# genome/breakdancer

Hardware: AMD Instinct MI355X
Metric: read-pairs/s, records resident in HBM -> scored SV table (SURVEY 8d timing i); end to end from BAM: config.timings.bam_to_table (vs_baseline is taken there) (higher is better)
Workload: dtype int32

## Files before the change

### breakdancer_amd/csrc/k2_compact.hip

```cpp
#include <cstdlib>

#include "bdx_dev.h"
#include "bdx_finalize.h"

namespace bdx {

size_t k2_lds_bytes(int) { return 0; }

constexpr int kSub = kK2TilesPerWave;
constexpr int kPerLane = 4 * kSub;
constexpr int kTile2 = kTile * kSub;
constexpr int kSlice = 256;
constexpr int kOffBits = 10;
static_assert(kPerLane <= 32 && kTile2 <= (1 << kOffBits), "K2 super tile");

__device__ __forceinline__ unsigned class_byte(const uint64_t (&cq)[kSub / 2], int r) {
    uint64_t v = cq[0];
#pragma unroll
    for (int q = 1; q < kSub / 2; ++q) v = (r >> 3) == q ? cq[q] : v;
    return (unsigned)((v >> (8 * (r & 7))) & 255u);
}

__device__ __forceinline__ void key_and_qlen_of(const K2Params& p, uint64_t i, uint64_t& key, int& qlen, uint64_t& check) {
    if (p.nseg == 0) {
// ... 156 lines not shown
                    const uint64_t i = (uint64_t)tile2 * kTile2 + (src & ((1u << kOffBits) - 1u));
                    const uint32_t j = rank0 + win + q;
                    const unsigned sam = p.r.flag[i];
                    p.c.tid[j] = p.r.tid[i];
                    p.c.pos[j] = p.r.pos[i];
                    p.c.isize[j] = abs(p.r.isize[i]);
                    uint64_t key, check = 0;
                    int qlen;
                    key_and_qlen_of(p, i, key, qlen, check);
                    p.c.meta[j] = meta_pack((int)((src >> kOffBits) & 15u), (sam >> 4) & 1u, lib_of(p, i), qlen);
                    p.c.key[j] = key;
                    if (p.c.check) p.c.check[j] = check;
                    p.c.idx[j] = (uint32_t)i;
                    p.c.nn[j] = s_nn[w * kSlice + q];
                }
            }
            __builtin_amdgcn_wave_barrier();
        }
        uint64_t kq[kSub / 2];
#pragma unroll
        for (int q = 0; q < kSub / 2; ++q) kq[q] = 0;
        if (nkeys > 1) {
#pragma unroll
            for (int r = 0; r < kPerLane; ++r)
                if (r < nvalid) kq[r >> 3] |= (uint64_t)(p.libs[lib_of(p, base + r)].key & 255) << (8 * (r & 7));
        }
        for (int k0 = 0; k0 < nkeys; k0 += 2) {
            uint32_t mk0 = 0, mk1 = 0;
            if (nkeys > 1) {
#pragma unroll
                for (int r = 0; r < kPerLane; ++r) {
                    const int key = (int)((kq[r >> 3] >> (8 * (r & 7))) & 255u);
                    if ((m_pk >> r) & 1u) { mk0 |= key == k0 ? 1u << r : 0u; mk1 |= key == k0 + 1 ? 1u << r : 0u; }
                }
            } else {
                mk0 = m_pk;
            }
            const uint32_t v = (uint32_t)__popc(mk0) + ((uint32_t)__popc(mk1) << 16);
            const uint32_t ex = wave_incl_scan(v) - v;
            const uint32_t b0 = k0 == 0 ? pre_k0 : col_prefix<kBases>(p, kColKey0 + k0, tile2, chunk, lane);
            const uint32_t b1 = k0 + 1 < nkeys ? (k0 == 0 ? pre_k1 : col_prefix<kBases>(p, kColKey0 + k0 + 1, tile2, chunk, lane)) : 0u;
            uint32_t j = rank0 + local0;
            for (uint32_t mm = m_anom; mm; mm &= mm - 1, ++j) {
                if (j >= p.c.cap) break;
                const int r = __builtin_ctz(mm);
                const uint32_t upto = (2u << r) - 1u;
                p.c.pk[(size_t)k0 * p.c.cap + j] = b0 + (ex & 0xFFFFu) + (uint32_t)__popc(mk0 & upto);
                if (k0 + 1 < nkeys) p.c.pk[(size_t)(k0 + 1) * p.c.cap + j] = b1 + (ex >> 16) + (uint32_t)__popc(mk1 & upto);
            }
        }
    }
}

__device__ __forceinline__ void k2_fills(const K2Params& p) {
#pragma nounroll
    for (int f = 0; f < 4; ++f)
        for (uint32_t i = blockIdx.x * kBlock + threadIdx.x; i < p.fill_words[f]; i += gridDim.x * kBlock) p.fill_ptr[f][i] = p.fill_value[f];
}

__global__ __launch_bounds__(kBlock) void k2_compact_kernel(const K2Params p) {
    k2_fills(p);
    k2_body<true>(p, gridDim.x);
}

__global__ __launch_bounds__(kBlock) void k2_compact_side_kernel(const K2Params p, const FinalizeParams fp) {
    k2_fills(p);
    if (blockIdx.x == gridDim.x - 1) {
        finalize2_body(fp);
        return;
    }
    k2_body<false>(p, gridDim.x - 1);
}

void launch_k2(const K2Params& p, size_t lds, hipStream_t s, const FinalizeParams* side) {
    const uint32_t ntiles2 = (p.ntiles + kSub - 1) / kSub;
    const uint32_t nblk = (ntiles2 + kWaves - 1) / kWaves;
    const uint32_t cap = 8192u;
    const uint32_t grid = nblk < cap ? nblk : cap;
    if (side) hipLaunchKernelGGL(k2_compact_side_kernel, dim3(grid + 1), dim3(kBlock), lds, s, p, *side);
    else hipLaunchKernelGGL(k2_compact_kernel, dim3(grid), dim3(kBlock), lds, s, p);
}

}

__global__ void k2_noop_kernel() {}
namespace bdx { void warm_k2(hipStream_t s) { hipLaunchKernelGGL(k2_noop_kernel, dim3(1), dim3(64), 0, s); } }
```

### breakdancer_amd/csrc/k4_join.hip

```cpp
#include "bdx_k3.h"
#include "bdx_scan.h"

namespace bdx {

__device__ __forceinline__ uint64_t mix64(uint64_t h) {
    h ^= h >> 33;
    h *= 0xff51afd7ed558ccdull;
    h ^= h >> 33;
    h *= 0xc4ceb9fe1a85ec53ull;
    h ^= h >> 33;
    return h;
}
__device__ __forceinline__ uint32_t bucket_of(uint64_t h, uint32_t log2b) { return log2b ? (uint32_t)(h >> (64 - log2b)) : 0u; }

constexpr int kPartChunk = 512;

__global__ __launch_bounds__(256) void k4_count_kernel(K4Arrays k4, Entries en, const uint32_t* n_ptr) {
    extern __shared__ __attribute__((aligned(16))) unsigned char smem[];
    uint32_t* s_h = (uint32_t*)smem;
    const uint32_t na = *n_ptr;
    const uint32_t base = blockIdx.x * kPartChunk;
    if (base >= na) return;
    for (uint32_t b = threadIdx.x; b < k4.nbuckets; b += 256) s_h[b] = 0;
    __syncthreads();
// ... 66 lines not shown
__device__ __forceinline__ void join_bucket(uint64_t* tkey, int32_t* tidx, uint32_t cap, const K4Arrays& k4, const int32_t* region,
                                            const uint64_t* check, uint32_t off, uint32_t cnt, StageCounts* counts) {
    for (uint32_t s = threadIdx.x; s < cap; s += blockDim.x) tidx[s] = -1;
    __syncthreads();
    for (uint32_t e = threadIdx.x; e < cnt; e += blockDim.x) {
        const uint64_t key = k4.e_key[off + e];
        const int32_t j = (int32_t)k4.e_idx[off + e];
        uint32_t s = (uint32_t)(mix64(key) & 0xffffffffu) % cap;
        uint32_t probes = 0;
        bool placed = true;
        while (atomicCAS(&tidx[s], -1, j) != -1) {
            s = s + 1 == cap ? 0 : s + 1;
            if (++probes > kMaxProbes) { placed = false; break; }
        }
        if (placed) tkey[s] = key;
        else counts->irregular = 1;
    }
    __syncthreads();
    for (uint32_t e = threadIdx.x; e < cnt; e += blockDim.x) {
        const uint64_t key = k4.e_key[off + e];
        const int32_t j = (int32_t)k4.e_idx[off + e];
        uint32_t s = (uint32_t)(mix64(key) & 0xffffffffu) % cap;
        int32_t mate = -1;
        const uint32_t lim = cap < kMaxProbes ? cap : kMaxProbes;
        for (uint32_t probes = 0; probes < lim; ++probes) {
            const int32_t o = tidx[s];
            if (o == -1) break;
            if (o != j && tkey[s] == key && (!check || check[o] == check[j])) {
                if (mate != -1) counts->irregular = 1;
                mate = o;
            }
            s = s + 1 == cap ? 0 : s + 1;
        }
        if (mate >= 0 && (region[j] < 0 || region[mate] < 0)) mate = -2;
        k4.partner[j] = mate;
    }
}

__global__ __launch_bounds__(256) void k4_join_kernel(K4Arrays k4, const int32_t* region, const uint64_t* check, StageCounts* counts) {
    extern __shared__ __attribute__((aligned(16))) unsigned char smem[];
    const uint32_t b = blockIdx.x;
    const uint32_t off = k4.boff[b], cnt = k4.boff[b + 1] - off;
    if (cnt == 0) return;
    if (2 * cnt <= (uint32_t)kJoinLdsSlots) {
        uint64_t* tkey = (uint64_t*)smem;
        int32_t* tidx = (int32_t*)(tkey + kJoinLdsSlots);
        join_bucket<true>(tkey, tidx, 2 * cnt, k4, region, check, off, cnt, counts);
    } else {
        join_bucket<false>(k4.t_key + 2 * (size_t)off, k4.t_idx + 2 * (size_t)off, 2 * cnt, k4, region, check, off, cnt, counts);
    }
}

constexpr uint32_t kJoinForwardBlocks = 32;
__global__ __launch_bounds__(256) void k4_direct_join_kernel(K4Arrays k4, Entries en, const uint32_t* n_ptr, StageCounts* counts) {
    const uint32_t na = *n_ptr;
    const uint32_t fwd = en.r_rec_host ? kJoinForwardBlocks : 0u;
    if (blockIdx.x < fwd) {
        const uint32_t nr = en.counts->n_regions;
        const uint32_t t = blockIdx.x * 256 + threadIdx.x, gsz = fwd * 256;
        constexpr uint32_t kw = sizeof(RegionRec) / 4;
        {
            const uint32_t words = nr * kw, quads = words / 4;
            const uint4* src = (const uint4*)en.r_rec_dev;
            uint4* dst = (uint4*)en.r_rec_host;
            for (uint32_t i = t; i < quads; i += gsz) dst[i] = src[i];
            if (t < words - quads * 4) ((uint32_t*)en.r_rec_host)[quads * 4 + t] = ((const uint32_t*)en.r_rec_dev)[quads * 4 + t];
        }
        {
            const uint32_t words = nr * (uint32_t)en.nkeys2, quads = words / 4;
            const uint4* src = (const uint4*)en.r_pk_dev;
            uint4* dst = (uint4*)en.r_pk_host;
            for (uint32_t i = t; i < quads; i += gsz) dst[i] = src[i];
            if (t < words - quads * 4) en.r_pk_host[quads * 4 + t] = en.r_pk_dev[quads * 4 + t];
        }
    }
    const uint32_t j = blockIdx.x < fwd ? 0xFFFFFFFFu : (blockIdx.x - fwd) * 256 + threadIdx.x;
    const uint32_t kp = (blockIdx.x - fwd) * 4 + (threadIdx.x >> 6);
    (void)kp;
    KPROF(kp, 0);
    KPROF(kp, 1);
    if (j >= na) return;
    const uint32_t nl = en.n_local ? *en.n_local : na;
    const bool jf = j >= nl;
    int rj;
    if (jf) {
        rj = en.fregion[j - nl];
    } else if (en.c_rid) {
        rj = en.c_rid[en.cand[j]];
        en.region_out[j] = rj;
        if (en.k6_scratch) {
            const size_t cap = en.scratch_cap;
            en.k6_scratch[j] = 0; en.k6_scratch[cap + j] = j; en.k6_scratch[2 * cap + j] = 0; en.k6_scratch[3 * cap + j] = 0;
            en.k6_scratch[4 * cap + j] = 0; en.k6_scratch[5 * cap + j] = 0;
        }
    } else {
        rj = en.region[j];
    }
    const uint64_t key = jf ? en.fkey[j - nl] : en.key[j];
    const uint64_t chk = en.check ? (jf ? en.fcheck[j - nl] : en.check[j]) : 0ull;
    const uint64_t h = mix64(key);
    if (key != 0x5555AAAA5555AAAAull) KPROF(kp, 2);
    const uint32_t tag = (uint32_t)(h >> 32);
    unsigned long long* table = (unsigned long long*)k4.t_key;
    const unsigned long long mine = ((unsigned long long)tag << 32) | j;
    uint32_t s = (uint32_t)h & k4.t_mask;
    for (uint32_t probes = 0; probes <= kMaxProbes; ++probes) {
        const unsigned long long old = atomicCAS(&table[s], ~0ull, mine);
        if (probes == 0 && old != 0x5555AAAA5555AAAAull) KPROF(kp, 3);
        if (old == ~0ull) return;
        if ((uint32_t)(old >> 32) == tag) {
            const uint32_t o = (uint32_t)old;
            const bool of = o >= nl;
            const uint64_t okey = of ? en.fkey[o - nl] : en.key[o];
            if (okey == key && (!en.check || (of ? en.fcheck[o - nl] : en.check[o]) == chk)) {
                const int ro = of ? en.fregion[o - nl] : (en.c_rid ? en.c_rid[en.cand[o]] : en.region[o]);
                const bool alive = rj >= 0 && ro >= 0;
                if (!jf) k4.partner[j] = alive ? (int32_t)o : -2;
                if (!of && atomicExch(&k4.partner[o], alive ? (int32_t)j : -2) != -1) counts->irregular = 1;
                if (alive && k4.pair_lo) {
                    if (jf != of) {
                        if (jf) k4.pair_lo[o] = rj; else k4.pair_lo[j] = ro;
                    } else if (!jf) {
                        if (o < j) k4.pair_lo[j] = ro;
                        else k4.pair_lo[o] = rj;
                    }
// ... 44 lines not shown
```

### breakdancer_amd/csrc/k6_assemble.hip

```cpp
#include <algorithm>
#include <cstdint>

#include "bdx_k3.h"

#include "bdx_insert.h"
#include "bdx_poisson.h"
#include "bdx_scan.h"

namespace bdx {

namespace {

__device__ __forceinline__ uint64_t readlane64(uint64_t v, int l) {
    const uint32_t lo = (uint32_t)__builtin_amdgcn_readlane((int)(uint32_t)v, l);
    const uint32_t hi = (uint32_t)__builtin_amdgcn_readlane((int)(uint32_t)(v >> 32), l);
    return ((uint64_t)hi << 32) | lo;
}

__device__ __forceinline__ uint32_t wave_sum_u32(uint32_t v) {
#pragma unroll
    for (int o = 32; o > 0; o >>= 1) v += __shfl_xor(v, o);
    return v;
}

// ... 38 lines not shown
        const uint32_t ct = kWeighted ? (uint32_t)__builtin_amdgcn_readlane((int)wc, t) : 1u;
        const bool eq = kt == key;
        m.cnt += eq ? ct : 0u;
        m.sum += eq ? st : 0u;
        eq_before += (eq && t < lane) ? 1u : 0u;
        m.gw += ((kt >> 12) == (key >> 12)) ? ct : 0u;
        if (kWeighted) {
            m.total += ct;
            m.wself += (uint32_t)(kt >> 12) == r ? ct : 0u;
        }
    }
    if (!kWeighted) {
        m.total = (uint32_t)__popcll(hasmask);
        m.wself = (uint32_t)__popcll(__ballot(has && (uint32_t)(key >> 12) == r));
    }
    m.leader = has && eq_before == 0;
    m.lmask = __ballot(m.leader);
    bool lo_first = true;
    for (uint64_t mm = m.lmask; mm; mm &= mm - 1) {
        const int t = __builtin_ctzll(mm);
        const uint64_t kt = readlane64(key, t);
        const bool same_lo = (kt >> 12) == (key >> 12);
        m.gparts += same_lo ? 1u : 0u;
        if (kt < key) {
            ++m.rank;
            if (same_lo) lo_first = false;
        }
    }
    m.gleader = m.leader && lo_first;
    return m;
}

__global__ __launch_bounds__(256) void k6_pairs_kernel(K6Arrays a) {
    __shared__ PartRec s_stash[4][64];
    const int lane = threadIdx.x & 63, w = threadIdx.x >> 6;
    const uint32_t nwaves = gridDim.x * 4;
    if (a.flag_regions && blockIdx.x == 0 && threadIdx.x == 0) {
        __threadfence_system();
        *(volatile uint32_t*)a.flag_regions = a.flag_value;
    }
    if (blockIdx.x == 0 && a.emit_part) a.emit_part[threadIdx.x] = 0;
    const uint32_t NR = a.counts->n_regions;
    const uint32_t mrp = (uint32_t)max(a.min_read_pair, 0);
    for (uint32_t r = blockIdx.x * 4 + (threadIdx.x >> 6); r < NR; r += nwaves) {
        const RegionRec rr = a.r_rec[r];
        const uint32_t first = a.first_of ? a.first_of[r] : rr.first, n = rr.n;
        RegSum rs{};
        auto load_read = [&](uint32_t c0, uint64_t& key, uint32_t& is) -> bool {
            const uint32_t i = c0 + lane;
            key = ~0ull;
            is = 0;
            if (i >= n) return false;
            const uint32_t j = first + i;
            int32_t plo;
            if (a.pair_lo) {
                plo = a.pair_lo[j];
            } else {
                const int32_t p = a.partner[j];
                plo = (p >= 0 && (uint32_t)p < j) ? a.region_of[p] : -1;
            }
            if (plo < 0) return false;
            const uint32_t m = a.meta[j];
            key = ((uint64_t)(uint32_t)plo << 12) | ((uint64_t)meta_lib(m) << 4) | (uint64_t)meta_flag(m);
            is = (uint32_t)a.isize[j];
            return true;
        };
        uint64_t key = ~0ull;
        uint32_t is = 0;
        bool has = false, merged = false;
        Merged m{};
        if (a.in_groups) {
            const uint32_t g0 = a.in_goff[r], ng = a.in_goff[r + 1] - g0;
            auto load_group = [&](uint32_t c0, uint64_t& k, uint32_t& cnt, uint32_t& sm) -> bool {
                const uint32_t i = c0 + lane;
                k = ~0ull; cnt = 0; sm = 0;
                if (i >= ng) return false;
                const GroupRec g = a.in_groups[g0 + i];
                k = ((g.key >> 38) << 12) | (g.key & 0xFFFull);
                cnt = g.pairs; sm = g.sum_isize;
                return true;
            };
            if (ng <= 64) {
                uint32_t cnt;
                has = load_group(0, key, cnt, is);
                if (__ballot(has)) {
                    m = merge_items<true>(key, cnt, is, has, r, lane);
                    merged = true;
                }
            } else {
                rs.big = 1u;
                for (uint32_t c0 = 0; c0 < ng; c0 += 64) {
                    uint64_t ck;
                    uint32_t cc, ci;
                    const bool ch = load_group(c0, ck, cc, ci);
                    const Merged cm = merge_items<true>(ck, cc, ci, ch, r, lane);
                    const uint32_t clo = (uint32_t)(ck >> 12);
                    rs.n_pairs += cm.total;
                    rs.w_self += cm.wself;
                    if (cm.gleader && clo < r) {
                        atomicAdd(&a.out_deg[clo], 1u);
                        a.bad_v[clo] = 1u;
                        if (a.taint && a.r_rec[clo].n == 0) { a.taint[clo] = 1; a.taint[r] = 1; }
                    }
                    if (lane == 0) a.bad_v[r] = 1u;
                    const uint32_t nl = (uint32_t)__popcll(cm.lmask);
                    uint32_t base = 0;
                    if (lane == 0) base = atomicAdd(&a.counts->n_groups, nl);
                    base = (uint32_t)__builtin_amdgcn_readfirstlane((int)base);
                    if (cm.leader) {
                        const uint32_t o = base + cm.rank;
                        if (o < a.g_cap) {
                            GroupRec g;
                            g.key = group_pack(clo, r, (uint32_t)((ck >> 4) & 255), (uint32_t)(ck & 15));
                            g.pairs = cm.cnt;
                            g.sum_isize = cm.sum;
                            a.g_rec[o] = g;
                        } else {
                            a.counts->overflow = 1;
// ... 24 lines not shown
            __builtin_amdgcn_wave_barrier();
            if (fits) {
                if (np) {
                    has = (uint32_t)lane < np;
                    const PartRec q = has ? s_stash[w][lane] : PartRec{~0ull, 0u, 0u};
                    key = q.key;
                    m = merge_items<true>(key, q.pairs, q.sum, has, r, lane);
                    merged = true;
                }
            } else {
                rs.big = 1u;
                for (uint32_t c0 = 0; c0 < n; c0 += 64) {
                    uint64_t ck;
                    uint32_t ci;
                    const bool ch = load_read(c0, ck, ci);
                    if (!__ballot(ch)) continue;
                    const Merged cm = merge_items<false>(ck, 1u, ci, ch, r, lane);
                    const uint32_t clo = (uint32_t)(ck >> 12);
                    rs.n_pairs += cm.total;
                    rs.w_self += cm.wself;
                    if (cm.gleader && clo < r) {
                        atomicAdd(&a.out_deg[clo], 1u);
                        a.bad_v[clo] = 1u;
                        if (a.taint && a.r_rec[clo].n == 0) { a.taint[clo] = 1; a.taint[r] = 1; }
                    }
                    if (lane == 0) a.bad_v[r] = 1u;
                    const uint32_t nl = (uint32_t)__popcll(cm.lmask);
                    uint32_t base = 0;
                    if (lane == 0) base = atomicAdd(&a.counts->n_groups, nl);
                    base = (uint32_t)__builtin_amdgcn_readfirstlane((int)base);
                    if (cm.leader) {
                        const uint32_t o = base + cm.rank;
                        if (o < a.g_cap) {
                            GroupRec g;
                            g.key = group_pack(clo, r, (uint32_t)((ck >> 4) & 255), (uint32_t)(ck & 15));
                            g.pairs = cm.cnt;
                            g.sum_isize = cm.sum;
                            a.g_rec[o] = g;
                        } else {
                            a.counts->overflow = 1;
                        }
                    }
                }
            }
            __builtin_amdgcn_wave_barrier();
        }
        if (merged) {
            const uint32_t lo = (uint32_t)(key >> 12);
            rs.n_pairs = m.total;
            rs.w_self = m.wself;
            const bool strong = m.gw >= mrp;
            const bool in_edge = m.gleader && lo < r && strong;
            const uint64_t gl_in = __ballot(in_edge);
            if (in_edge) atomicAdd(&a.out_deg[lo], 1u);
            if (a.taint && in_edge && a.r_rec[lo].n == 0) { a.taint[lo] = 1; a.taint[r] = 1; }
            rs.np_all = (uint32_t)__popcll(m.lmask);
            rs.np_self = (uint32_t)__popcll(__ballot(m.leader && lo == r));
            rs.np_emit = (uint32_t)__popcll(__ballot(m.leader && (lo == r || strong)));
            rs.n_weak = (uint32_t)__popcll(__ballot(m.gleader && lo < r && !strong));
            rs.n_in = (uint32_t)__popcll(gl_in);
            if (rs.n_in > (uint32_t)kK6MaxIn) {
                if (in_edge) a.bad_v[lo] = 1u;
                if (lane == 0) a.bad_v[r] = 1u;
            } else {
                if (in_edge && !a.force_host) {
                    const uint32_t lr = a.label[r], ll = a.label[lo];
                    if (lr < ll) atomicMin(&a.label[lo], lr);
                    else if (ll < lr) atomicMin(&a.label[r], ll);
                }
                uint64_t mm = gl_in;
#pragma unroll
                for (int e = 0; e < kK6MaxIn; ++e) {
                    if (mm) {
                        const int t = __builtin_ctzll(mm);
                        mm &= mm - 1;
                        rs.e_lo[e] = (uint32_t)__builtin_amdgcn_readlane((int)lo, t);
                        rs.e_w[e] = (uint32_t)__builtin_amdgcn_readlane((int)m.gw, t);
                        rs.e_off[e] = (uint32_t)__builtin_amdgcn_readlane((int)m.rank, t);
                        rs.e_cnt[e] = (uint32_t)__builtin_amdgcn_readlane((int)m.gparts, t);
                    }
                }
            }
            if (m.leader) a.parts[first + m.rank] = PartRec{(lo < r && !strong) ? (key | kWeakPart) : key, m.cnt, m.sum};
        }
        if (lane == 0) a.rs[r] = rs;
    }
}

__global__ __launch_bounds__(256) void k6_label_kernel(K6Arrays a) {
    const uint32_t r = blockIdx.x * blockDim.x + threadIdx.x;
    if (r >= a.counts->n_regions) return;
    const RegSum* s = &a.rs[r];
    const uint32_t n_in = s->n_in;
    if (s->big || n_in == 0 || n_in > (uint32_t)kK6MaxIn) return;
    for (uint32_t e = 0; e < n_in; ++e) {
        const uint32_t lo = s->e_lo[e];
        const uint32_t lr = a.label[r], ll = a.label[lo];
        if (lr < ll) atomicMin(&a.label[lo], lr);
        else if (ll < lr) atomicMin(&a.label[r], ll);
    }
    const uint32_t l = a.label[r], l2 = a.label[l];
    if (l2 < l) atomicMin(&a.label[r], l2);
}

__global__ __launch_bounds__(256) void k6_classify_kernel(K6Arrays a) {
    const uint32_t r = blockIdx.x * blockDim.x + threadIdx.x;
    if (r >= a.counts->n_regions) return;
    const RegSum* s = &a.rs[r];
    const uint32_t n_in = s->n_in;
    const bool hub = s->big || n_in > (uint32_t)kK6MaxIn;
    if (!hub && n_in == 0 && a.out_deg[r] == 0 && s->np_self == 0) return;
    const uint32_t L = a.label[r];
    if (hub || a.bad_v[r] || (a.taint && a.taint[r])) a.bad[L] = 1u;
    if (!hub) {
#pragma unroll
        for (uint32_t e = 0; e < (uint32_t)kK6MaxIn; ++e) {
            if (e < n_in) {
                const uint32_t ll = a.label[s->e_lo[e]];
                if (ll != L) { a.bad[L] = 1u; a.bad[ll] = 1u; }
            }
        }
    }
    const uint32_t slot = atomicAdd(&a.mcount[L], 1u);
    if (a.big_walk && slot < (uint32_t)kK6BigMembers) a.member_ids[(size_t)L * kK6BigMembers + slot] = r;
    if (slot < (uint32_t)kK6MaxMembers) {
        static_assert(sizeof(MemberInfo) == 7 * 16 && sizeof(RegionRec) == 36 && offsetof(MemberInfo, rec) == 4 && offsetof(MemberInfo, np_all) == 40 &&
                          offsetof(MemberInfo, e_lo) == 56 && offsetof(MemberInfo, stored) == 104, "a member's record is seven 16-byte words");
        const uint32_t* rw = (const uint32_t*)&a.r_rec[r];
        const uint32_t r0 = rw[0], r1 = rw[1], r2 = rw[2], r3 = rw[3], r4 = rw[4], r5 = rw[5], r6 = rw[6], r7 = rw[7], r8 = a.first_of ? a.first_of[r] : rw[8];
        const uint32_t stored = (int)(a.chr_restricted ? r5 : r3) >= a.min_read_pair ? 1u : 0u;
        uint4* dst = (uint4*)&a.members[(size_t)L * kK6MaxMembers + slot];
        dst[0] = make_uint4(r, r0, r1, r2);
        dst[1] = make_uint4(r3, r4, r5, r6);
        dst[2] = make_uint4(r7, r8, s->np_all, s->np_self);
        dst[3] = make_uint4(s->w_self, hub ? 0u : n_in, s->e_lo[0], s->e_lo[1]);
        dst[4] = make_uint4(s->e_lo[2], s->e_w[0], s->e_w[1], s->e_w[2]);
        dst[5] = make_uint4(s->e_off[0], s->e_off[1], s->e_off[2], s->e_cnt[0]);
        dst[6] = make_uint4(s->e_cnt[1], s->e_cnt[2], stored, 0u);
    }
    if (s->np_emit) atomicAdd(&a.pcount[L], s->np_emit);
}

namespace {

struct RunConst {
    const float* lib_mean;
    const uint32_t* hist;
    const float* key_density;
    uint32_t covered;
};

constexpr int kFewLibs = 4;
__device__ bool assemble_sv(const K6Arrays& a, const RunConst& rc_, const PartRec* P, uint32_t A, int32_t B, const RegionRec& ra, const RegionRec& rb,
                            const uint32_t* pk_last_a, const uint32_t* pk_first_b, const GrpRange (&gs)[3], int max_readlen,
                            uint32_t slot, uint32_t start, bool store, uint32_t* nacc_out, uint32_t* ncn_out, uint32_t kprow = ~0u) {
    (void)kprow;
    KPROF(kprow, 0);
    const uint32_t lib_room = a.lib_stride;
    const int mrp = a.min_read_pair;
    int cv[kNumFlags];
#pragma unroll
    for (int f = 0; f < kNumFlags; ++f) cv[f] = 0;
    int num_pairs = 0;
    const PartRec none_part{0ull, 0u, 0u};
#pragma unroll
    for (int g = 0; g < 3; ++g)
        for (uint32_t i = 0; i < gs[g].cnt; i += 4) {
            PartRec q[4];
#pragma unroll
            for (int u = 0; u < 4; ++u) q[u] = i + u < gs[g].cnt ? P[gs[g].beg + i + u] : none_part;
#pragma unroll
            for (int u = 0; u < 4; ++u) {
                const int f = (int)(q[u].key & 15);
                const int pr = (int)q[u].pairs;
#pragma unroll
                for (int ff = 0; ff < kNumFlags; ++ff) cv[ff] += f == ff ? pr : 0;
                num_pairs += pr;
            }
        }
    if (num_pairs != 0x7FFFFFFF) KPROF(kprow, 1);
    if (num_pairs < mrp) return false;
    int flag = BDX_NA, flag_count;
    {
        int best = 0, bestv = cv[0];
#pragma unroll
        for (int f = 1; f < kNumFlags; ++f)
            if (cv[f] > bestv) { best = f; bestv = cv[f]; }
        if (bestv > 0) flag = best;
        flag_count = bestv > 0 ? bestv : cv[BDX_NA];
    }
    if (flag_count < mrp) return false;

    int chr[2], pos[2], fwd[2], rev[2];
// ... 86 lines not shown
        for (int k = 0; k < nk; ++k) {
            const uint32_t cnt = pk_first_b[k] - pk_last_a[k];
            if (cnt == 0) continue;
            const float cn = __fmul_rn(__fdiv_rn((float)cnt, __fmul_rn(rc_.key_density[k], span)), 2.0f);
            if (store) cs[ncn] = CnStage{k, cn};
            ++ncn;
            cn_sum = __fadd_rn(cn_sum, cn);
        }
    }
    const float allele_frequency =
        ncn ? __fsub_rn(1.0f, __fdiv_rn(cn_sum, __fmul_rn(2.0f, (float)ncn))) : __uint_as_float(0xFFC00000u);

    if (ncn != 0x7FFFFFFFu) KPROF(kprow, 3);
    if (flag != BDX_ARP_RF && flag != BDX_ARP_RR && pos[0] + max_readlen - 5 < pos[1]) pos[0] += max_readlen - 5;
    const int diffspan = (int)((double)__fdiv_rn(diff, (float)flag_count) + 0.5);

    SvOut o;
    for (int i = 0; i < 2; ++i) { o.sv.chr[i] = chr[i]; o.sv.pos[i] = pos[i] + 1; o.sv.fwd[i] = fwd[i]; o.sv.rev[i] = rev[i]; }
    o.sv.flag = flag; o.sv.size = diffspan; o.sv.score = 0; o.sv.num_reads = flag_count; o.sv.printed = 0;
    o.sv.region[0] = (int32_t)A; o.sv.region[1] = B;
    o.sv.lib_begin = 0; o.sv.lib_count = (int32_t)nacc;
    o.sv.cn_begin = 0; o.sv.cn_count = (int32_t)ncn;
    o.sv.allele_frequency = allele_frequency; o.sv.logp = 0.0;
    o.grp_mask = (gs[0].cnt ? 1u : 0u) | (gs[1].cnt ? 2u : 0u) | (gs[2].cnt ? 4u : 0u);
    o.start = start;
    if (store) a.sv_stage[slot] = o;
    KPROF(kprow, 4);
    *nacc_out = nacc;
    *ncn_out = ncn;
    return true;
}

__device__ __forceinline__ int pair_index(int x, int y) {
    return x == 0 ? y - 1 : (x == 1 ? y + 1 : 5);
}

}

namespace {

__device__ __forceinline__ bool component_on_device(const K6Arrays& a, uint32_t L) {
    return !a.force_host && !a.bad[L] && a.mcount[L] <= (uint32_t)(a.big_walk ? kK6BigMembers : kK6MaxMembers) &&
           min((uint32_t)a.nlibs, a.pcount[L]) <= a.lib_stride;
}

}

__global__ __launch_bounds__(256) void k6_emit_kernel(K6Arrays a) {
    const int lane = threadIdx.x & 63;
    const uint32_t NR = a.counts->n_regions;
    const uint32_t r = blockIdx.x * blockDim.x + threadIdx.x;
    const bool active = r < NR;
    RegSum s{};
    uint32_t od = 0, L = 0;
    if (active) { s = a.rs[r]; od = a.out_deg[r]; L = a.label[r]; a.own_nsv[r] = 0; a.own_nacc[r] = 0; a.own_ncn[r] = 0; }
    const bool hub = s.big || s.n_in > (uint32_t)kK6MaxIn;
    const bool registered = active && (hub || s.n_in > 0 || od > 0 || s.np_self > 0);
    const bool covered = registered && component_on_device(a, L);
    {
        const uint32_t need = (registered && !covered && !s.big) ? s.np_emit : 0u;
        uint32_t o = wave_reserve(need, &a.counts->n_groups);
        if (need) {
            const uint32_t first = a.first_of ? a.first_of[r] : a.r_rec[r].first;
            for (uint32_t i = 0; i < s.np_all; ++i) {
                const PartRec q = a.parts[first + i];
                const uint64_t key = q.key;
                if (key & kWeakPart) continue;
                if (o < a.g_cap) {
                    GroupRec g;
                    g.key = ((key >> 12) << 38) | ((uint64_t)r << 12) | (key & 0xFFFull);
                    g.pairs = q.pairs;
                    g.sum_isize = q.sum;
                    a.g_rec[o] = g;
                } else {
                    a.counts->overflow = 1;
                }
                ++o;
            }
        }
    }
    {
        const bool owner = covered && L == r;
        const bool small = owner && a.mcount[L] <= (uint32_t)kK6MaxMembers;
        if (active) a.owners[r] = small ? a.mcount[L] : 0u;
        const uint32_t no = (uint32_t)__popcll(__ballot(small));
        uint32_t* part = a.emit_part ? a.emit_part + (blockIdx.x & 63u) * 4 : nullptr;
        if (lane == 0 && no) atomicAdd(part ? &part[0] : &a.counts->n_owners, no);
        const uint32_t ob = wave_reserve(owner && !small ? 1u : 0u, &a.counts->n_owners_big);
        if (owner && !small) a.owners_big[ob] = r;
    }
    {
        const uint32_t pairs = active ? s.n_pairs : 0u;
        const uint32_t grp = (active ? s.n_weak : 0u) + (covered ? s.n_in + (s.np_self ? 1u : 0u) : 0u);
        const uint32_t gb = (covered && a.mcount[L] > (uint32_t)kK6MaxMembers) ? s.n_in + (s.np_self ? 1u : 0u) : 0u;
        const uint32_t tp = wave_sum_u32(pairs), tg = wave_sum_u32(grp), tb = wave_sum_u32(gb);
        if (lane == 0) {
            uint32_t* part = a.emit_part ? a.emit_part + (blockIdx.x & 63u) * 4 : nullptr;
            if (tp) atomicAdd(part ? &part[1] : &a.counts->n_pairs, tp);
            if (tg) atomicAdd(part ? &part[2] : &a.counts->n_groups_dev, tg);
            if (tb) atomicAdd(part ? &part[3] : &a.counts->n_groups_big, tb);
        }
    }
}

namespace {
__device__ __forceinline__ uint32_t mirrored_count_word(const K6Arrays& a, int lane) {
    constexpr int kWords = (int)(sizeof(StageCounts) / 4);
    uint32_t v = lane < kWords ? ((const uint32_t*)a.counts)[lane] : 0u;
    if (a.emit_part) {
        uint32_t p0 = a.emit_part[lane * 4], p1 = a.emit_part[lane * 4 + 1], p2 = a.emit_part[lane * 4 + 2], p3 = a.emit_part[lane * 4 + 3];
        p0 = wave_sum_u32(p0); p1 = wave_sum_u32(p1); p2 = wave_sum_u32(p2); p3 = wave_sum_u32(p3);
        constexpr int iOwners = (int)(offsetof(StageCounts, n_owners) / 4), iPairs = (int)(offsetof(StageCounts, n_pairs) / 4),
                      iDev = (int)(offsetof(StageCounts, n_groups_dev) / 4), iBig = (int)(offsetof(StageCounts, n_groups_big) / 4);
        v += lane == iOwners ? p0 : lane == iPairs ? p1 : lane == iDev ? p2 : lane == iBig ? p3 : 0u;
    }
    return v;
}
}

__global__ __launch_bounds__(64) void k6_mirror_kernel(K6Arrays a) {
    const uint32_t word = mirrored_count_word(a, (int)threadIdx.x);
    if (threadIdx.x < sizeof(StageCounts) / 4) ((uint32_t*)a.counts_host)[threadIdx.x] = word;
    if (a.flag_groups) {
        __threadfence_system();
        __syncthreads();
        if (threadIdx.x == 0) *(volatile uint32_t*)a.flag_groups = a.flag_value;
    }
}

struct BigTab {
    uint32_t rid[kK6BigMembers];
    RegionRec rec[kK6BigMembers];
    RegSum rs[kK6BigMembers];
    uint8_t elo[kK6BigMembers][4];
    int tails[4 * kK6BigMembers], newtails[4 * kK6BigMembers];
};

__device__ __forceinline__ void walk_big(const K6Arrays& a, BigTab& B, uint32_t L, int lane, uint32_t NR) {
    const int k = (int)a.mcount[L];
    const int mrp = a.min_read_pair, nk = a.nkeys;
    const uint32_t period = (uint32_t)a.period;
    const RunConst rc_{a.lib_mean, a.hist, a.key_density, a.p1->covered_ref_len};
    {
        const uint32_t id = lane < k ? a.member_ids[(size_t)L * kK6BigMembers + lane] : 0xffffffffu;
        uint32_t rank = 0;
        for (int q = 0; q < k; ++q) rank += (uint32_t)__shfl((int)id, q) < id ? 1u : 0u;
        if (lane < k) B.rid[rank] = id;
    }
    __builtin_amdgcn_wave_barrier();
    constexpr int kRecW = sizeof(RegionRec) / 4, kRsW = sizeof(RegSum) / 4;
    for (int i = lane; i < k * (kRecW + kRsW); i += 64) {
        const int m = i / (kRecW + kRsW), wd = i - m * (kRecW + kRsW);
        const uint32_t r = B.rid[m];
        if (wd < kRecW) ((uint32_t*)&B.rec[m])[wd] = (wd == kRecW - 1 && a.first_of) ? a.first_of[r] : ((const uint32_t*)&a.r_rec[r])[wd];
// ... 466 lines not shown
    }
    if (!valid || !e.x) return;
    uint32_t lb = ex_l + a.ins_pre_l[hb1], cb = ex_c + a.ins_pre_c[hb1], slot = slot0;
    for (uint32_t q = 0; q < e.x; ++q) {
        const uint32_t pos = ex_sv + hb1 + q;
        a.sv_src[pos] = slot;
        a.sv_begin[pos] = make_uint2(lb, cb);
        if (a.sv_vx) a.sv_vx[pos] = j;
        if (q + 1 < e.x) {
            lb += (uint32_t)a.sv_stage[slot].sv.lib_count;
            cb += (uint32_t)a.sv_stage[slot].sv.cn_count;
            slot = a.slot_next[slot];
        }
    }
}

__global__ __launch_bounds__(kScanBlock) void k6_score_kernel(K6Arrays a, double ln10, int score_threshold, int with_scores) {
    __shared__ uint32_t s_rec[kScanBlock / 64][64 * kSvWords];
    __shared__ uint32_t s_fromw[kScanBlock / 64][64];
    __shared__ uint32_t s_printed;
    const uint32_t tid = threadIdx.x;
    const int lane = tid & 63, w = tid >> 6;
    const uint32_t bid = blockIdx.x;
    const uint32_t kp = 32768u + 16384u + (bid * 4 + w < 16384u ? bid * 4 + w : 16383u);
    (void)kp;
    KPROF(kp, 0);
    if (tid == 0) s_printed = 0;
    __syncthreads();
    const uint32_t n_sv = a.counts->overflow ? 0u : a.counts->n_sv_dev;
    for (uint32_t c0 = (bid * (kScanBlock / 64) + (uint32_t)w) * 64u; c0 < n_sv; c0 += gridDim.x * kScanBlock) {
        const uint32_t cnt = min(64u, n_sv - c0);
        const bool act = (uint32_t)lane < cnt;
        uint32_t* rec = s_rec[w];
        const uint32_t from = act ? a.sv_src[c0 + lane] : 0u;
        const uint2 bg = act ? a.sv_begin[c0 + lane] : make_uint2(0u, 0u);
        s_fromw[w][lane] = from;
        __builtin_amdgcn_wave_barrier();
        for (uint32_t i = lane; i < cnt * kSvWords; i += 64) {
            const uint32_t sv = i / kSvWords, wd = i - sv * kSvWords;
            const uint32_t f = s_fromw[w][sv];
            const uint32_t* src = (f & 0x80000000u) ? (const uint32_t*)(a.hs_rec + (f & 0x7FFFFFFFu)) : (const uint32_t*)(a.sv_stage + f);
            rec[i] = src[wd];
        }
        __builtin_amdgcn_wave_barrier();
        KPROF(kp, 3);
        SvOut* o = (SvOut*)rec + (act ? lane : 0);
        const bool hosted = (from & 0x80000000u) != 0;
        const int32_t nl = act ? o->sv.lib_count : 0, ncn = act ? o->sv.cn_count : 0;
        const int32_t l0 = o->sv.lib_begin, k0 = o->sv.cn_begin;
        if (act) { o->sv.lib_begin = (int32_t)bg.x; o->sv.cn_begin = (int32_t)bg.y; }
        int32_t max_nl = nl, max_ncn = ncn;
#pragma unroll
        for (int off = 32; off > 0; off >>= 1) { max_nl = max(max_nl, __shfl_xor(max_nl, off)); max_ncn = max(max_ncn, __shfl_xor(max_ncn, off)); }
        double logp = 0.0, err = 0.0;
        for (int32_t q = 0; q < max_nl; ++q) {
            const bool a2 = q < nl;
            double lam = 1.0;
            int32_t k = 0, li = 0;
            if (a2) {
                if (hosted) { lam = a.hs_lambda[l0 + q]; k = a.hs_lib_pairs[l0 + q]; li = a.hs_lib_index[l0 + q]; }
                else { const LibStage t = a.lib_stage[(size_t)from * a.lib_stride + q]; lam = t.lambda; k = t.rc; li = t.lib; }
            }
            const double lt = poisson_term(lam, k, a2, lane);
            if (a2) {
                a.lib_index[bg.x + q] = li;
                a.lib_pairs[bg.x + q] = k;
                if (a.ltail_host) a.ltail_host[bg.x + q] = lt;
                const double tmp_a = __dsub_rn(lt, err);
                const double tmp_b = __dadd_rn(logp, tmp_a);
                err = __dsub_rn(__dsub_rn(tmp_b, logp), tmp_a);
                logp = tmp_b;
            }
        }
        for (int32_t t = 0; t < max_ncn; ++t) {
            if (t < ncn) {
                int32_t key;
                float value;
                if (hosted) { key = a.hs_cn_key[k0 + t]; value = a.hs_cn_value[k0 + t]; }
                else { const CnStage cn = a.cn_stage[(size_t)from * a.nkeys + t]; key = cn.key; value = cn.value; }
                a.cn_key[bg.y + t] = key;
                a.cn_value[bg.y + t] = value;
            }
        }
        bool pr = false;
        if (act && with_scores) {
            const double phred_tmp = __ddiv_rn(__dmul_rn(-10.0, logp), ln10);
            const double r = __dadd_rn(phred_tmp, 0.5);
            int phred;
            if (phred_tmp > 99.0) phred = 99;
            else if (r != r || r >= 2147483648.0 || r <= -2147483649.0) phred = INT32_MIN;
            else phred = (int)r;
            pr = phred > score_threshold;
            o->sv.logp = logp;
            o->sv.score = phred;
            o->sv.printed = pr ? 1 : 0;
        }
        if (a.sv_key && act) {
            const unsigned long long T = a.sv_vx[c0 + lane], st = o->start;
            a.sv_key[c0 + lane] = (T << kKeyShiftT) | (T == st ? 1ull << 33 : 0ull) | (st << kKeyShiftStart);
        }
        const uint32_t npr = (uint32_t)__popcll(__ballot(pr));
        if (lane == 0 && npr) atomicAdd(&s_printed, npr);
        KPROF(kp, 4);
        __builtin_amdgcn_wave_barrier();
        if (a.wire_rows) {
            SvWire wr{};
            if (act) {
                wr.pos[0] = o->sv.pos[0]; wr.pos[1] = o->sv.pos[1]; wr.region[0] = o->sv.region[0]; wr.region[1] = o->sv.region[1];
                wr.size = o->sv.size; wr.score = o->sv.score; wr.num_reads = o->sv.num_reads; wr.allele_frequency = o->sv.allele_frequency;
                wr.logp = o->sv.logp; wr.start = o->start;
                wr.bits = ((uint32_t)o->sv.lib_count & 255u) | (((uint32_t)o->sv.cn_count & 255u) << 8) | (((uint32_t)o->sv.flag & 15u) << 16) |
                          ((o->grp_mask & 7u) << 20) | ((o->sv.printed ? 1u : 0u) << 23);
            }
            __builtin_amdgcn_wave_barrier();
            if (act) {
                uint32_t* q = rec + lane * kWireWords;
                const uint32_t* src = (const uint32_t*)&wr;
#pragma unroll
                for (int k = 0; k < kWireWords; ++k) q[k] = src[k];
            }
            __builtin_amdgcn_wave_barrier();
            uint32_t* dst = (uint32_t*)a.sv_out + (size_t)c0 * kWireWords;
            for (uint32_t i = lane; i < cnt * kWireWords; i += 64) dst[i] = rec[i];
        } else {
            uint32_t* dst = (uint32_t*)(a.sv_out + c0);
            for (uint32_t i = lane; i < cnt * kSvWords; i += 64) dst[i] = rec[i];
        }
        __builtin_amdgcn_wave_barrier();
    }
    __syncthreads();
    if (tid == 0) {
        if (s_printed) atomicAdd(&a.counts->n_printed, s_printed);
// ... 86 lines not shown
```

Measured before the change: 29.02 billion.

## Vectorize fills, software-pipeline copies and loads across k2, k4 and k6 kernels

K2 fills now write 16-byte quads, and the side kernel's finalize block no longer takes part in the fills. The K4 forward copy to host memory keeps four loads in flight ahead of the stores. Several K6 kernels hoist or batch their global loads: classify reads the region summary by value and issues all label loads up front, the group emit loop reads parts four at a time as uint4, and the assemble loop prefetches the next lib and copy-number entries while computing the current one. Together these aim to hide memory latency, at the cost of more registers and some redundant clamped loads.

Result: faster. 29.60 billion (median of 6 runs) (+2.0%).

```diff
diff --git a/breakdancer_amd/csrc/k2_compact.hip b/breakdancer_amd/csrc/k2_compact.hip
--- a/breakdancer_amd/csrc/k2_compact.hip
+++ b/breakdancer_amd/csrc/k2_compact.hip
@@ -232,23 +232,27 @@
     }
 }
 
-__device__ __forceinline__ void k2_fills(const K2Params& p) {
+__device__ __forceinline__ void k2_fills(const K2Params& p, uint32_t nblk) {
 #pragma nounroll
-    for (int f = 0; f < 4; ++f)
-        for (uint32_t i = blockIdx.x * kBlock + threadIdx.x; i < p.fill_words[f]; i += gridDim.x * kBlock) p.fill_ptr[f][i] = p.fill_value[f];
+    for (int f = 0; f < 4; ++f) {
+        const uint32_t words = p.fill_words[f], quads = words >> 2, v = p.fill_value[f];
+        uint4* const q = (uint4*)p.fill_ptr[f];
+        for (uint32_t i = blockIdx.x * kBlock + threadIdx.x; i < quads; i += nblk * kBlock) q[i] = make_uint4(v, v, v, v);
+        if (blockIdx.x == 0 && threadIdx.x < (words & 3u)) p.fill_ptr[f][4 * quads + threadIdx.x] = v;
+    }
 }
 
 __global__ __launch_bounds__(kBlock) void k2_compact_kernel(const K2Params p) {
-    k2_fills(p);
+    k2_fills(p, gridDim.x);
     k2_body<true>(p, gridDim.x);
 }
 
 __global__ __launch_bounds__(kBlock) void k2_compact_side_kernel(const K2Params p, const FinalizeParams fp) {
-    k2_fills(p);
     if (blockIdx.x == gridDim.x - 1) {
         finalize2_body(fp);
         return;
     }
+    k2_fills(p, gridDim.x - 1);
     k2_body<false>(p, gridDim.x - 1);
 }
 
diff --git a/breakdancer_amd/csrc/k4_join.hip b/breakdancer_amd/csrc/k4_join.hip
--- a/breakdancer_amd/csrc/k4_join.hip
+++ b/breakdancer_amd/csrc/k4_join.hip
@@ -142,6 +142,23 @@
 }
 
 constexpr uint32_t kJoinForwardBlocks = 32;
+constexpr uint32_t kJoinForwardAhead = 4;
+
+__device__ __forceinline__ void forward_quads(uint4* dst, const uint4* src, uint32_t quads, uint32_t t, uint32_t gsz) {
+    if (quads == 0) return;
+    static_assert(kJoinForwardAhead == 4, "four named words (an array of them is kept in scratch memory)");
+    const uint32_t last = quads - 1u;
+    uint4 c0 = src[min(t, last)], c1 = src[min(t + gsz, last)], c2 = src[min(t + 2 * gsz, last)], c3 = src[min(t + 3 * gsz, last)];
+    uint32_t i = t;
+    for (; i + 3 * gsz < quads; i += 4 * gsz) {
+        const uint4 n0 = src[min(i + 4 * gsz, last)], n1 = src[min(i + 5 * gsz, last)], n2 = src[min(i + 6 * gsz, last)], n3 = src[min(i + 7 * gsz, last)];
+        dst[i] = c0; dst[i + gsz] = c1; dst[i + 2 * gsz] = c2; dst[i + 3 * gsz] = c3;
+        c0 = n0; c1 = n1; c2 = n2; c3 = n3;
+    }
+    if (i < quads) dst[i] = c0;
+    if (i + gsz < quads) dst[i + gsz] = c1;
+    if (i + 2 * gsz < quads) dst[i + 2 * gsz] = c2;
+}
 __global__ __launch_bounds__(256) void k4_direct_join_kernel(K4Arrays k4, Entries en, const uint32_t* n_ptr, StageCounts* counts) {
     const uint32_t na = *n_ptr;
     const uint32_t fwd = en.r_rec_host ? kJoinForwardBlocks : 0u;
@@ -151,16 +168,12 @@
         constexpr uint32_t kw = sizeof(RegionRec) / 4;
         {
             const uint32_t words = nr * kw, quads = words / 4;
-            const uint4* src = (const uint4*)en.r_rec_dev;
-            uint4* dst = (uint4*)en.r_rec_host;
-            for (uint32_t i = t; i < quads; i += gsz) dst[i] = src[i];
+            forward_quads((uint4*)en.r_rec_host, (const uint4*)en.r_rec_dev, quads, t, gsz);
             if (t < words - quads * 4) ((uint32_t*)en.r_rec_host)[quads * 4 + t] = ((const uint32_t*)en.r_rec_dev)[quads * 4 + t];
         }
         {
             const uint32_t words = nr * (uint32_t)en.nkeys2, quads = words / 4;
-            const uint4* src = (const uint4*)en.r_pk_dev;
-            uint4* dst = (uint4*)en.r_pk_host;
-            for (uint32_t i = t; i < quads; i += gsz) dst[i] = src[i];
+            forward_quads((uint4*)en.r_pk_host, (const uint4*)en.r_pk_dev, quads, t, gsz);
             if (t < words - quads * 4) en.r_pk_host[quads * 4 + t] = en.r_pk_dev[quads * 4 + t];
         }
     }
diff --git a/breakdancer_amd/csrc/k6_assemble.hip b/breakdancer_amd/csrc/k6_assemble.hip
--- a/breakdancer_amd/csrc/k6_assemble.hip
+++ b/breakdancer_amd/csrc/k6_assemble.hip
@@ -114,6 +114,7 @@
             is = 0;
             if (i >= n) return false;
             const uint32_t j = first + i;
+            const uint32_t m = a.meta[j], isz = (uint32_t)a.isize[j];
             int32_t plo;
             if (a.pair_lo) {
                 plo = a.pair_lo[j];
@@ -121,11 +122,10 @@
                 const int32_t p = a.partner[j];
                 plo = (p >= 0 && (uint32_t)p < j) ? a.region_of[p] : -1;
             }
-            if (plo < 0) return false;
-            const uint32_t m = a.meta[j];
-            key = ((uint64_t)(uint32_t)plo << 12) | ((uint64_t)meta_lib(m) << 4) | (uint64_t)meta_flag(m);
-            is = (uint32_t)a.isize[j];
-            return true;
+            const bool ok = plo >= 0;
+            key = ok ? ((uint64_t)(uint32_t)plo << 12) | ((uint64_t)meta_lib(m) << 4) | (uint64_t)meta_flag(m) : ~0ull;
+            is = ok ? isz : 0u;
+            return ok;
         };
         uint64_t key = ~0ull;
         uint32_t is = 0;
@@ -256,7 +256,6 @@
             const bool strong = m.gw >= mrp;
             const bool in_edge = m.gleader && lo < r && strong;
             const uint64_t gl_in = __ballot(in_edge);
-            if (in_edge) atomicAdd(&a.out_deg[lo], 1u);
             if (a.taint && in_edge && a.r_rec[lo].n == 0) { a.taint[lo] = 1; a.taint[r] = 1; }
             rs.np_all = (uint32_t)__popcll(m.lmask);
             rs.np_self = (uint32_t)__popcll(__ballot(m.leader && lo == r));
@@ -285,6 +284,7 @@
                     }
                 }
             }
+            if (in_edge) atomicAdd(&a.out_deg[lo], 1u);
             if (m.leader) a.parts[first + m.rank] = PartRec{(lo < r && !strong) ? (key | kWeakPart) : key, m.cnt, m.sum};
         }
         if (lane == 0) a.rs[r] = rs;
@@ -310,39 +310,40 @@
 __global__ __launch_bounds__(256) void k6_classify_kernel(K6Arrays a) {
     const uint32_t r = blockIdx.x * blockDim.x + threadIdx.x;
     if (r >= a.counts->n_regions) return;
-    const RegSum* s = &a.rs[r];
-    const uint32_t n_in = s->n_in;
-    const bool hub = s->big || n_in > (uint32_t)kK6MaxIn;
-    if (!hub && n_in == 0 && a.out_deg[r] == 0 && s->np_self == 0) return;
-    const uint32_t L = a.label[r];
-    if (hub || a.bad_v[r] || (a.taint && a.taint[r])) a.bad[L] = 1u;
-    if (!hub) {
-#pragma unroll
-        for (uint32_t e = 0; e < (uint32_t)kK6MaxIn; ++e) {
-            if (e < n_in) {
-                const uint32_t ll = a.label[s->e_lo[e]];
-                if (ll != L) { a.bad[L] = 1u; a.bad[ll] = 1u; }
-            }
-        }
-    }
+    const RegSum s = a.rs[r];
+    const uint32_t od = a.out_deg[r], L = a.label[r], bv = a.bad_v[r], tn = a.taint ? a.taint[r] : 0u;
+    const uint32_t* rw = (const uint32_t*)&a.r_rec[r];
+    const uint32_t r0 = rw[0], r1 = rw[1], r2 = rw[2], r3 = rw[3], r4 = rw[4], r5 = rw[5], r6 = rw[6], r7 = rw[7], r8 = a.first_of ? a.first_of[r] : rw[8];
+    const uint32_t n_in = s.n_in;
+    const bool hub = s.big || n_in > (uint32_t)kK6MaxIn;
+    if (!hub & (n_in == 0) & (od == 0) & (s.np_self == 0)) return;
+    const bool own_bad = hub | (bv != 0) | (tn != 0);
+    uint32_t ll[kK6MaxIn];
+#pragma unroll
+    for (uint32_t e = 0; e < (uint32_t)kK6MaxIn; ++e) {
+        const uint32_t lo = (!hub && e < n_in) ? s.e_lo[e] : r;
+        ll[e] = a.label[lo];
+    }
+    if (own_bad) a.bad[L] = 1u;
+#pragma unroll
+    for (uint32_t e = 0; e < (uint32_t)kK6MaxIn; ++e)
+        if (ll[e] != L) { a.bad[L] = 1u; a.bad[ll[e]] = 1u; }
     const uint32_t slot = atomicAdd(&a.mcount[L], 1u);
     if (a.big_walk && slot < (uint32_t)kK6BigMembers) a.member_ids[(size_t)L * kK6BigMembers + slot] = r;
     if (slot < (uint32_t)kK6MaxMembers) {
         static_assert(sizeof(MemberInfo) == 7 * 16 && sizeof(RegionRec) == 36 && offsetof(MemberInfo, rec) == 4 && offsetof(MemberInfo, np_all) == 40 &&
                           offsetof(MemberInfo, e_lo) == 56 && offsetof(MemberInfo, stored) == 104, "a member's record is seven 16-byte words");
-        const uint32_t* rw = (const uint32_t*)&a.r_rec[r];
-        const uint32_t r0 = rw[0], r1 = rw[1], r2 = rw[2], r3 = rw[3], r4 = rw[4], r5 = rw[5], r6 = rw[6], r7 = rw[7], r8 = a.first_of ? a.first_of[r] : rw[8];
         const uint32_t stored = (int)(a.chr_restricted ? r5 : r3) >= a.min_read_pair ? 1u : 0u;
         uint4* dst = (uint4*)&a.members[(size_t)L * kK6MaxMembers + slot];
         dst[0] = make_uint4(r, r0, r1, r2);
         dst[1] = make_uint4(r3, r4, r5, r6);
-        dst[2] = make_uint4(r7, r8, s->np_all, s->np_self);
-        dst[3] = make_uint4(s->w_self, hub ? 0u : n_in, s->e_lo[0], s->e_lo[1]);
-        dst[4] = make_uint4(s->e_lo[2], s->e_w[0], s->e_w[1], s->e_w[2]);
-        dst[5] = make_uint4(s->e_off[0], s->e_off[1], s->e_off[2], s->e_cnt[0]);
-        dst[6] = make_uint4(s->e_cnt[1], s->e_cnt[2], stored, 0u);
-    }
-    if (s->np_emit) atomicAdd(&a.pcount[L], s->np_emit);
+        dst[2] = make_uint4(r7, r8, s.np_all, s.np_self);
+        dst[3] = make_uint4(s.w_self, hub ? 0u : n_in, s.e_lo[0], s.e_lo[1]);
+        dst[4] = make_uint4(s.e_lo[2], s.e_w[0], s.e_w[1], s.e_w[2]);
+        dst[5] = make_uint4(s.e_off[0], s.e_off[1], s.e_off[2], s.e_cnt[0]);
+        dst[6] = make_uint4(s.e_cnt[1], s.e_cnt[2], stored, 0u);
+    }
+    if (s.np_emit) atomicAdd(&a.pcount[L], s.np_emit);
 }
 
 namespace {
@@ -535,8 +536,8 @@
     const uint32_t r = blockIdx.x * blockDim.x + threadIdx.x;
     const bool active = r < NR;
     RegSum s{};
-    uint32_t od = 0, L = 0;
-    if (active) { s = a.rs[r]; od = a.out_deg[r]; L = a.label[r]; a.own_nsv[r] = 0; a.own_nacc[r] = 0; a.own_ncn[r] = 0; }
+    uint32_t od = 0, L = 0, own_members = 0;
+    if (active) { s = a.rs[r]; od = a.out_deg[r]; L = a.label[r]; }
     const bool hub = s.big || s.n_in > (uint32_t)kK6MaxIn;
     const bool registered = active && (hub || s.n_in > 0 || od > 0 || s.np_self > 0);
     const bool covered = registered && component_on_device(a, L);
@@ -545,27 +546,35 @@
         uint32_t o = wave_reserve(need, &a.counts->n_groups);
         if (need) {
             const uint32_t first = a.first_of ? a.first_of[r] : a.r_rec[r].first;
-            for (uint32_t i = 0; i < s.np_all; ++i) {
-                const PartRec q = a.parts[first + i];
-                const uint64_t key = q.key;
-                if (key & kWeakPart) continue;
-                if (o < a.g_cap) {
-                    GroupRec g;
-                    g.key = ((key >> 12) << 38) | ((uint64_t)r << 12) | (key & 0xFFFull);
-                    g.pairs = q.pairs;
-                    g.sum_isize = q.sum;
-                    a.g_rec[o] = g;
-                } else {
-                    a.counts->overflow = 1;
-                }
-                ++o;
+            static_assert(sizeof(PartRec) == 16 && offsetof(PartRec, pairs) == 8 && offsetof(PartRec, sum) == 12, "a part is one 16-byte word");
+            const uint4* const P4 = (const uint4*)a.parts;
+            for (uint32_t i = 0; i < s.np_all; i += 4) {
+                uint4 q[4];
+#pragma unroll
+                for (int u = 0; u < 4; ++u) q[u] = P4[first + min(i + u, s.np_all - 1u)];
+#pragma unroll
+                for (int u = 0; u < 4; ++u) {
+                    const uint64_t key = (uint64_t)q[u].x | ((uint64_t)q[u].y << 32);
+                    if (i + u >= s.np_all || (key & kWeakPart)) continue;
+                    if (o < a.g_cap) {
+                        GroupRec g;
+                        g.key = ((key >> 12) << 38) | ((uint64_t)r << 12) | (key & 0xFFFull);
+                        g.pairs = q[u].z;
+                        g.sum_isize = q[u].w;
+                        a.g_rec[o] = g;
+                    } else {
+                        a.counts->overflow = 1;
+                    }
+                    ++o;
+                }
             }
         }
     }
     {
         const bool owner = covered && L == r;
-        const bool small = owner && a.mcount[L] <= (uint32_t)kK6MaxMembers;
-        if (active) a.owners[r] = small ? a.mcount[L] : 0u;
+        const uint32_t mc = owner ? a.mcount[L] : 0u;
+        const bool small = owner && mc <= (uint32_t)kK6MaxMembers;
+        own_members = small ? mc : 0u;
         const uint32_t no = (uint32_t)__popcll(__ballot(small));
         uint32_t* part = a.emit_part ? a.emit_part + (blockIdx.x & 63u) * 4 : nullptr;
         if (lane == 0 && no) atomicAdd(part ? &part[0] : &a.counts->n_owners, no);
@@ -583,6 +592,10 @@
             if (tg) atomicAdd(part ? &part[2] : &a.counts->n_groups_dev, tg);
             if (tb) atomicAdd(part ? &part[3] : &a.counts->n_groups_big, tb);
         }
+    }
+    if (active) {
+        a.owners[r] = own_members;
+        a.own_nsv[r] = 0; a.own_nacc[r] = 0; a.own_ncn[r] = 0;
     }
 }
 
@@ -1155,15 +1168,31 @@
         int32_t max_nl = nl, max_ncn = ncn;
 #pragma unroll
         for (int off = 32; off > 0; off >>= 1) { max_nl = max(max_nl, __shfl_xor(max_nl, off)); max_ncn = max(max_ncn, __shfl_xor(max_ncn, off)); }
+        auto load_term = [&](int32_t q, double& lam, int32_t& k, int32_t& li) {
+            lam = 1.0; k = 0; li = 0;
+            if (q < nl) {
+                if (hosted) { lam = a.hs_lambda[l0 + q]; k = a.hs_lib_pairs[l0 + q]; li = a.hs_lib_index[l0 + q]; }
+                else { const LibStage t = a.lib_stage[(size_t)from * a.lib_stride + q]; lam = t.lambda; k = t.rc; li = t.lib; }
+            }
+        };
+        auto load_cn = [&](int32_t t, int32_t& key, float& value) {
+            key = 0; value = 0.f;
+            if (t < ncn) {
+                if (hosted) { key = a.hs_cn_key[k0 + t]; value = a.hs_cn_value[k0 + t]; }
+                else { const CnStage cn = a.cn_stage[(size_t)from * a.nkeys + t]; key = cn.key; value = cn.value; }
+            }
+        };
+        double lam_n;
+        int32_t k_n, li_n, key_n;
+        float value_n;
+        load_term(0, lam_n, k_n, li_n);
+        load_cn(0, key_n, value_n);
         double logp = 0.0, err = 0.0;
         for (int32_t q = 0; q < max_nl; ++q) {
             const bool a2 = q < nl;
-            double lam = 1.0;
-            int32_t k = 0, li = 0;
-            if (a2) {
-                if (hosted) { lam = a.hs_lambda[l0 + q]; k = a.hs_lib_pairs[l0 + q]; li = a.hs_lib_index[l0 + q]; }
-                else { const LibStage t = a.lib_stage[(size_t)from * a.lib_stride + q]; lam = t.lambda; k = t.rc; li = t.lib; }
-            }
+            const double lam = lam_n;
+            const int32_t k = k_n, li = li_n;
+            load_term(q + 1, lam_n, k_n, li_n);
             const double lt = poisson_term(lam, k, a2, lane);
             if (a2) {
                 a.lib_index[bg.x + q] = li;
@@ -1176,11 +1205,10 @@
             }
         }
         for (int32_t t = 0; t < max_ncn; ++t) {
+            const int32_t key = key_n;
+            const float value = value_n;
+            load_cn(t + 1, key_n, value_n);
             if (t < ncn) {
-                int32_t key;
-                float value;
-                if (hosted) { key = a.hs_cn_key[k0 + t]; value = a.hs_cn_value[k0 + t]; }
-                else { const CnStage cn = a.cn_stage[(size_t)from * a.nkeys + t]; key = cn.key; value = cn.value; }
                 a.cn_key[bg.y + t] = key;
                 a.cn_value[bg.y + t] = value;
             }
```
